# octavian-ganea/equidock_public

Measured on NVIDIA H100. Metric: protein_pairs_per_sec_iegmn_fwd_kabsch, higher is better.
Workload: dtype f32

## Files before the change

### equidock_public_b200/csrc/attn_tc.cu

```cuda
#include "tc_common.cuh"

namespace eqd {

#ifdef ATTN_PROF
__device__ long long g_attn_prof[16];
#define PROF_MARK(k) do { if (tid == 0 && blockIdx.x == 0) { const long long t_ = clock64(); prof_acc[k] += t_ - prof_t; prof_t = t_; } } while (0)
#else
#define PROF_MARK(k) do { } while (0)
#endif

#define AT_THREADS 256
#define AT_KEYS 64
#define AT_CHUNK_BYTES 8192
#define AT_A_SPLIT 16384
#define AT_LD 68

struct AtGroupSmem {
  unsigned char k[2][3][AT_CHUNK_BYTES];
  unsigned char v[2][3][AT_CHUNK_BYTES];
  float red[EQD_TM * 2];
  float x5c[2][AT_KEYS * 16];
  float red5[EQD_TM * 2 * 5];
};
struct AtSmem {
  unsigned char qa[3 * AT_A_SPLIT];
  unsigned char pa[3 * AT_A_SPLIT];
  AtGroupSmem grp;
  unsigned long long k_bar[2], v_bar[2];
};

__global__ void __launch_bounds__(AT_THREADS, 1)
attention0_tc_kernel(eqd_graph g, const float* __restrict__ proj, int pw, const unsigned char* __restrict__ kv,
                    long kv_split_stride, const float* __restrict__ x5, float* __restrict__ mu, int ldmu) {
  extern __shared__ __align__(128) unsigned char smem_raw[];
  AtSmem& S = *reinterpret_cast<AtSmem*>(smem_raw);
  const int tid = threadIdx.x, q = tid, half = q >> 7, r = q & 127, wgi = tid >> 7;
  AtGroupSmem& G = S.grp;
  TRACE_START(1);
  if (tid == 0) {
    for (int b = 0; b < 2; ++b) {
      mbar_init(&S.k_bar[b], 1);
      mbar_init(&S.v_bar[b], 1);
    }
    asm volatile("fence.mbarrier_init.release.cluster;" ::: "memory");
  }
  if (q == 0) TRACE_PHASE(1, blockIdx.x, 0, 14);
  __syncthreads();
  if (q == 0) TRACE_PHASE(1, blockIdx.x, 0, 13);
  const unsigned k_saddr = smem_u32(G.k), v_saddr = smem_u32(G.v);
  const unsigned qa_saddr = smem_u32(S.qa), pa_saddr = smem_u32(S.pa);
  float* const dtile = reinterpret_cast<float*>(S.pa);
  unsigned kph[2] = {0, 0}, vph[2] = {0, 0};
  const int B = g.n_pairs;
  const unsigned char* k_g = kv;
  const unsigned char* v_g = kv + 3 * kv_split_stride;

  auto load_chunk = [&](const unsigned char* src, unsigned char (*dst)[AT_CHUNK_BYTES], unsigned long long* bar, int blk0,
                        int x5buf) {
    if (q == 0) {
      const bool with5 = x5buf >= 0;
      mbar_expect_tx(bar, 3 * AT_CHUNK_BYTES + (with5 ? AT_KEYS * 64 : 0));
#pragma unroll
      for (int s = 0; s < 3; ++s) bulk_g2s(dst[s], src + s * kv_split_stride + (long)blk0 * 1024, AT_CHUNK_BYTES, bar);
      if (with5) bulk_g2s(G.x5c[x5buf], x5 + (long)blk0 * 8 * 16, AT_KEYS * 64, bar);
    }
  };
  auto add_s5 = [&](float (&s)[32], const float* xc, const float (&q5)[5]) {
#pragma unroll
    for (int i = 0; i < 32; ++i) {
      const float* row = xc + (half * 32 + i) * 16;
      const float4 k4 = *reinterpret_cast<const float4*>(row);
      const float k8 = row[8];
      s[i] += q5[0] * k4.x + q5[1] * k4.y + q5[2] * k4.z + q5[3] * k4.w + q5[4] * k8;
    }
  };
  auto gemm_s = [&](int kb_, bool hi_only) {
    float d[32];
    wg_gemm6<64>(d, [&](int sp, int kb) { return a_desc_at<EQD_TM>(qa_saddr, AT_A_SPLIT, wgi, sp, kb); },
                 [&](int sp, int kk) { return b_desc_ex(k_saddr + (kb_ * 3 + sp) * AT_CHUNK_BYTES + kk * 256, 128, 1024); },
                 4, false, hi_only);
    wg_store_d<64>(dtile + wgi * 64 * AT_LD, AT_LD, d, tid & 127);
  };
  auto gemm_pv = [&](int vb_) {
    float d[32];
    wg_gemm6<64, 1>(d, [&](int sp, int kb) { return a_desc_at<EQD_TM>(pa_saddr, AT_A_SPLIT, wgi, sp, kb); },
                    [&](int sp, int kk) { return b_desc_ex(v_saddr + (vb_ * 3 + sp) * AT_CHUNK_BYTES + kk * 2048, 1024, 128); },
                    4, false);
    __syncthreads();
    wg_store_d<64>(dtile + wgi * 64 * AT_LD, AT_LD, d, tid & 127);
  };

#ifdef ATTN_PROF
  __shared__ long long prof_acc[16];
  long long prof_t = clock64();
  if (tid == 0)
    for (int k = 0; k < 16; ++k) prof_acc[k] = 0;
#endif
  for (int tile = blockIdx.x; tile < g.n_node_tiles; tile += gridDim.x) {
    PROF_MARK(15);
    if (q == 0) TRACE_PHASE(1, blockIdx.x, tile, 1);
    const int seg = g.node_tiles[2 * tile], node0 = g.node_tiles[2 * tile + 1];
    const int nvalid = min(EQD_TM, g.seg_ptr[seg + 1] - node0);
    const int pseg = seg < B ? seg + B : seg - B;
    const int j0 = g.seg_ptr[pseg], j1 = g.seg_ptr[pseg + 1];
    const int blk_lo = j0 >> 3, blk_hi = (j1 + 7) >> 3;
    const int nchunks = (blk_hi - blk_lo + 7) >> 3;
    const int node = node0 + r;
    const bool valid = r < nvalid;
    PROF_MARK(0);
    if (nchunks > 0) load_chunk(k_g, G.k[0], &S.k_bar[0], blk_lo, 0);
    float q5[5] = {0.f, 0.f, 0.f, 0.f, 0.f};
    if (valid) {
#pragma unroll
      for (int e = 0; e < 5; ++e) q5[e] = x5[(long)node * 16 + 10 + e];
    }
    {
      float v[32];
      const float4* sp = reinterpret_cast<const float4*>(proj + (long)node * pw + 128 + half * 32);
#pragma unroll
      for (int c4 = 0; c4 < 8; ++c4) {
        float4 t = valid ? sp[c4] : make_float4(0.f, 0.f, 0.f, 0.f);
        v[c4 * 4] = t.x; v[c4 * 4 + 1] = t.y; v[c4 * 4 + 2] = t.z; v[c4 * 4 + 3] = t.w;
      }
      store_half_split3<EQD_TM>(S.qa, AT_A_SPLIT, r, half * 32, v);
    }
    tc_fence_before();
    __syncthreads();
    PROF_MARK(1);
    float mx = -INFINITY;
    for (int c = 0; c < nchunks; ++c) {
      const int kb_ = c & 1;
      if (q == 0) TRACE_PHASE(1, blockIdx.x, tile, (c << 4) | 2);
      mbar_wait(&S.k_bar[kb_], kph[kb_]);
      kph[kb_] ^= 1;
      PROF_MARK(2);
      if (c + 1 < nchunks) load_chunk(k_g, G.k[kb_ ^ 1], &S.k_bar[kb_ ^ 1], blk_lo + 8 * (c + 1), kb_ ^ 1);
      else load_chunk(k_g, G.k[kb_ ^ 1], &S.k_bar[kb_ ^ 1], blk_lo, kb_ ^ 1);
      if (q == 0) TRACE_PHASE(1, blockIdx.x, tile, (c << 4) | 3);
      gemm_s(kb_, true);
      __syncthreads();
      PROF_MARK(3);
      float s[32];
      tile_ld32f(dtile, AT_LD, r, half * 32, s);
      add_s5(s, G.x5c[kb_], q5);
      const int key0 = (blk_lo + 8 * c) * 8 + half * 32;
#pragma unroll
      for (int i = 0; i < 32; ++i) {
        int kn = key0 + i;
        mx = fmaxf(mx, (kn >= j0 && kn < j1) ? s[i] : -INFINITY);
      }
      __syncthreads();
      PROF_MARK(4);
    }
    G.red[r * 2 + half] = mx;
    __syncthreads();
    mx = fmaxf(G.red[r * 2], G.red[r * 2 + 1]);
    float l = 0.f;
    float o_acc[32];
#pragma unroll
    for (int i = 0; i < 32; ++i) o_acc[i] = 0.f;
    if (nchunks > 0) load_chunk(v_g, G.v[0], &S.v_bar[0], blk_lo, -1);
    float o5[5] = {0.f, 0.f, 0.f, 0.f, 0.f};
    for (int c = 0; c < nchunks; ++c) {
      const int kb_ = (nchunks + c) & 1, vb_ = c & 1;
      if (q == 0) TRACE_PHASE(1, blockIdx.x, tile, (c << 4) | 4);
      mbar_wait(&S.k_bar[kb_], kph[kb_]);
      kph[kb_] ^= 1;
      PROF_MARK(5);
      if (c + 1 < nchunks) {
        load_chunk(k_g, G.k[kb_ ^ 1], &S.k_bar[kb_ ^ 1], blk_lo + 8 * (c + 1), kb_ ^ 1);
        load_chunk(v_g, G.v[vb_ ^ 1], &S.v_bar[vb_ ^ 1], blk_lo + 8 * (c + 1), -1);
      }
      if (q == 0) TRACE_PHASE(1, blockIdx.x, tile, (c << 4) | 5);
      gemm_s(kb_, false);
      __syncthreads();
      PROF_MARK(6);
      float s[32];
      tile_ld32f(dtile, AT_LD, r, half * 32, s);
      add_s5(s, G.x5c[kb_], q5);
      const int key0 = (blk_lo + 8 * c) * 8 + half * 32;
      float l4[4] = {0.f, 0.f, 0.f, 0.f};
#pragma unroll
      for (int i = 0; i < 32; ++i) {
        int kn = key0 + i;
        float pj = (kn >= j0 && kn < j1) ? expf(s[i] - mx) : 0.f;
        s[i] = pj;
        l4[i & 3] += pj;
        {
          const float* row = G.x5c[kb_] + (half * 32 + i) * 16;
          const float4 v4 = *reinterpret_cast<const float4*>(row + 4);
          o5[0] = fmaf(pj, v4.x, o5[0]);
          o5[1] = fmaf(pj, v4.y, o5[1]);
          o5[2] = fmaf(pj, v4.z, o5[2]);
          o5[3] = fmaf(pj, v4.w, o5[3]);
          o5[4] = fmaf(pj, row[9], o5[4]);
        }
      }
      l += (l4[0] + l4[1]) + (l4[2] + l4[3]);
      PROF_MARK(7);
      __syncthreads();
      PROF_MARK(8);
      store_half_split3<EQD_TM>(S.pa, AT_A_SPLIT, r, half * 32, s);
      tc_fence_before();
      __syncthreads();
      PROF_MARK(9);
      if (q == 0) TRACE_PHASE(1, blockIdx.x, tile, (c << 4) | 6);
      mbar_wait(&S.v_bar[vb_], vph[vb_]);
      vph[vb_] ^= 1;
      gemm_pv(vb_);
      __syncthreads();
      if (q == 0) TRACE_PHASE(1, blockIdx.x, tile, (c << 4) | 7);
      PROF_MARK(10);
      {
        float oc[32];
        tile_ld32f(dtile, AT_LD, r, half * 32, oc);
#pragma unroll
        for (int i = 0; i < 32; ++i) o_acc[i] += oc[i];
      }
      __syncthreads();
      PROF_MARK(11);
    }
    G.red[r * 2 + half] = l;
    {
#pragma unroll
      for (int e = 0; e < 5; ++e) G.red5[(r * 2 + half) * 5 + e] = o5[e];
    }
    __syncthreads();
    l = G.red[r * 2] + G.red[r * 2 + 1];
    {
      const float inv = l > 0.f ? 1.f / l : 0.f;
      if (valid && half == 0) {
        float e8[8];
#pragma unroll
        for (int e = 0; e < 5; ++e) e8[e] = (G.red5[r * 10 + e] + G.red5[r * 10 + 5 + e]) * inv;
        e8[5] = e8[6] = e8[7] = 0.f;
        float4* de = reinterpret_cast<float4*>(mu + (long)node * ldmu + 64);
        de[0] = make_float4(e8[0], e8[1], e8[2], e8[3]);
        de[1] = make_float4(e8[4], e8[5], e8[6], e8[7]);
      }
      if (valid) {
        float4* dst = reinterpret_cast<float4*>(mu + (long)node * ldmu + half * 32);
#pragma unroll
        for (int c4 = 0; c4 < 8; ++c4)
          dst[c4] = make_float4(o_acc[c4 * 4] * inv, o_acc[c4 * 4 + 1] * inv, o_acc[c4 * 4 + 2] * inv, o_acc[c4 * 4 + 3] * inv);
      }
    }
    __syncthreads();
    PROF_MARK(12);
  }
#ifdef ATTN_PROF
  if (tid == 0 && blockIdx.x == 0)
    for (int k = 0; k < 16; ++k) g_attn_prof[k] = prof_acc[k];
#endif
  if (q == 0) TRACE_PHASE(1, blockIdx.x, 0xffff, 15);
  TRACE_END(1);
}

#define AT_CHAINS 2

struct __align__(128) AtChainSmem {
  unsigned char k[2][3][AT_CHUNK_BYTES];
  unsigned char v[2][3][AT_CHUNK_BYTES];
  float qs[64 * 64];
  unsigned long long k_bar[2], v_bar[2];
};

struct AtTile {
  int node0, nvalid;
  int j0, j1;
  int blk_lo, nchunks;
};

__global__ void __launch_bounds__(AT_CHAINS * 128, 1)
attention64_tc_kernel(eqd_graph g, const float* __restrict__ proj, const unsigned char* __restrict__ kv,
                      long kv_split_stride, float* __restrict__ mu) {
  extern __shared__ __align__(128) unsigned char smem_raw[];
  AtChainSmem& W = reinterpret_cast<AtChainSmem*>(smem_raw)[threadIdx.x >> 7];
  const int tid = threadIdx.x, wgi = tid >> 7, t = tid & 127, lane = t & 31;
  const int bar = 1 + wgi;
  TRACE_START(1);
  if (t == 0) {
    for (int b = 0; b < 2; ++b) {
      mbar_init(&W.k_bar[b], 1);
      mbar_init(&W.v_bar[b], 1);
    }
    asm volatile("fence.mbarrier_init.release.cluster;" ::: "memory");
  }
  wg_barrier(bar);
  const unsigned k_saddr = smem_u32(W.k), v_saddr = smem_u32(W.v);
  const int B = g.n_pairs, nht = 2 * g.n_node_tiles, hstride = gridDim.x * AT_CHAINS;
  const unsigned char* k_g = kv;
  const unsigned char* v_g = kv + 3 * kv_split_stride;

  const int chain = blockIdx.x * AT_CHAINS + wgi;
  auto find_tile = [&](int k, AtTile& m) {
    for (; chain + k * hstride < nht; ++k) {
      const int ht = (chain + k * hstride) ^ (k & 1);
      const int seg = __ldg(g.node_tiles + 2 * (ht >> 1));
      m.node0 = __ldg(g.node_tiles + 2 * (ht >> 1) + 1) + 64 * (ht & 1);
      m.nvalid = min(64, __ldg(g.seg_ptr + seg + 1) - m.node0);
      if (m.nvalid <= 0) continue;
      const int pseg = seg < B ? seg + B : seg - B;
      m.j0 = __ldg(g.seg_ptr + pseg);
      m.j1 = __ldg(g.seg_ptr + pseg + 1);
      m.blk_lo = m.j0 >> 3;
      m.nchunks = (((m.j1 + 7) >> 3) - m.blk_lo + 7) >> 3;
      return k;
    }
    return -1;
  };
  unsigned kfill = 0, kcons = 0, vfill = 0, vcons = 0;
  auto fill = [&](unsigned char (*dst)[3][AT_CHUNK_BYTES], unsigned long long* bars, unsigned& n, const unsigned char* src,
                  int blk0) {
    if (t == 0) {
      unsigned long long* b = &bars[n & 1];
      mbar_expect_tx(b, 3 * AT_CHUNK_BYTES);
#pragma unroll
      for (int s = 0; s < 3; ++s) bulk_g2s(dst[n & 1][s], src + s * kv_split_stride + (long)blk0 * 1024, AT_CHUNK_BYTES, b);
    }
    ++n;
  };
  auto consume = [&](unsigned long long* bars, unsigned& n) {
    mbar_wait(&bars[n & 1], (n >> 1) & 1);
    return (int)((n++) & 1);
  };
  auto stage_q = [&](const AtTile& m) { stage_rows64(W.qs, proj, 320, 128, m.node0, m.nvalid, t); };

  const int fr0 = (t >> 5) * 16 + (lane >> 2), fc = 2 * (lane & 3);
  AtTile cur, nxt;
  int kt = find_tile(0, cur);
  bool k_ahead = false, v_ahead = false;
  if (kt >= 0) stage_q(cur);
  while (kt >= 0) {
    if (t == 0) TRACE_PHASE(1, chain, kt, 1);
    int ktn = -1;
    bool looked = false;
    auto look_ahead = [&]() {
      if (looked) return;
      looked = true;
      ktn = find_tile(kt + 1, nxt);
      if (ktn >= 0) stage_q(nxt);
    };
    if (cur.nchunks > 0 && !k_ahead) fill(W.k, W.k_bar, kfill, k_g, cur.blk_lo);
    cp_async_wait<0>();
    wg_barrier(bar);
    unsigned qf[3][4][4];
    staged_rows_to_a_split3(W.qs, t, qf);
    wg_barrier(bar);
    auto k_desc = [&](int kb_) {
      return [&, kb_](int sp, int kk) { return b_desc_ex(k_saddr + (kb_ * 3 + sp) * AT_CHUNK_BYTES + kk * 256, 128, 1024); };
    };
    float mx[2] = {-INFINITY, -INFINITY};
    for (int c = 0; c < cur.nchunks; ++c) {
      const int kb_ = consume(W.k_bar, kcons);
      fill(W.k, W.k_bar, kfill, k_g, cur.blk_lo + (c + 1 < cur.nchunks ? 8 * (c + 1) : 0));
      float s[32];
      wg_gemm6_rs_issue<64, 4, 0, true>(s, qf, k_desc(kb_), false);
      look_ahead();
      wg_mma_wait(s);
      const int key0 = (cur.blk_lo + 8 * c) * 8 + fc;
#pragma unroll
      for (int j = 0; j < 8; ++j)
#pragma unroll
        for (int e = 0; e < 2; ++e) {
          const int kn = key0 + 8 * j + e;
          const bool ok = kn >= cur.j0 && kn < cur.j1;
#pragma unroll
          for (int h = 0; h < 2; ++h) mx[h] = fmaxf(mx[h], ok ? s[4 * j + 2 * h + e] : -INFINITY);
        }
      wg_barrier(bar);
    }
    look_ahead();
#pragma unroll
    for (int h = 0; h < 2; ++h) {
      mx[h] = fmaxf(mx[h], __shfl_xor_sync(0xffffffffu, mx[h], 1));
      mx[h] = fmaxf(mx[h], __shfl_xor_sync(0xffffffffu, mx[h], 2));
    }
    float lh[2][2] = {{0.f, 0.f}, {0.f, 0.f}};
    float o_acc[32];
#pragma unroll
    for (int i = 0; i < 32; ++i) o_acc[i] = 0.f;
    if (cur.nchunks > 0 && !v_ahead) fill(W.v, W.v_bar, vfill, v_g, cur.blk_lo);
    for (int c = 0; c < cur.nchunks; ++c) {
      const int kb_ = consume(W.k_bar, kcons);
      const bool last = c + 1 == cur.nchunks;
      if (!last) {
        fill(W.k, W.k_bar, kfill, k_g, cur.blk_lo + 8 * (c + 1));
        fill(W.v, W.v_bar, vfill, v_g, cur.blk_lo + 8 * (c + 1));
      } else if (ktn >= 0 && nxt.nchunks > 0) {
        fill(W.k, W.k_bar, kfill, k_g, nxt.blk_lo);
        fill(W.v, W.v_bar, vfill, v_g, nxt.blk_lo);
      }
      float s[32];
      wg_gemm6_rs_issue<64, 4>(s, qf, k_desc(kb_), false);
      wg_mma_wait(s);
      const int key0 = (cur.blk_lo + 8 * c) * 8 + fc;
#pragma unroll
      for (int j = 0; j < 8; ++j)
#pragma unroll
        for (int e = 0; e < 2; ++e) {
          const int kn = key0 + 8 * j + e;
          const bool ok = kn >= cur.j0 && kn < cur.j1;
#pragma unroll
          for (int h = 0; h < 2; ++h) {
            float& x = s[4 * j + 2 * h + e];
            x = ok ? expf(x - mx[h]) : 0.f;
          }
        }
      {
        float ps[32];
#pragma unroll
        for (int i = 0; i < 32; ++i) ps[i] = __shfl_xor_sync(0xffffffffu, s[i], 2);
#pragma unroll
        for (int h = 0; h < 2; ++h)
#pragma unroll
          for (int ch = 0; ch < 2; ++ch) {
            float s0 = 0.f, s1 = 0.f;
#pragma unroll
            for (int c4 = 0; c4 < 8; ++c4) {
              s0 = __fadd_rn(s0, chain_val(s, ps, h, ch, c4, 0));
              s1 = __fadd_rn(s1, chain_val(s, ps, h, ch, c4, 1));
            }
            const float sp = __fadd_rn(s0, s1);
            lh[h][ch] = __fadd_rn(lh[h][ch], __fadd_rn(sp, __shfl_xor_sync(0xffffffffu, sp, 1)));
          }
      }
      unsigned pf[3][4][4];
      acc_to_a_split3<4>(s, pf);
      const int vb_ = consume(W.v_bar, vcons);
      float o[32];
      wg_gemm6_rs_issue<64, 4, 1>(o, pf, [&](int sp, int kk) {
        return b_desc_ex(v_saddr + (vb_ * 3 + sp) * AT_CHUNK_BYTES + kk * 2048, 1024, 128); }, false);
      wg_mma_wait(o);
#pragma unroll
      for (int i = 0; i < 32; ++i) o_acc[i] = __fadd_rn(o_acc[i], o[i]);
      wg_barrier(bar);
    }
    k_ahead = v_ahead = ktn >= 0 && nxt.nchunks > 0 && cur.nchunks > 0;
#pragma unroll
    for (int h = 0; h < 2; ++h) {
      const float l = __fadd_rn(lh[h][0], lh[h][1]);
      const float inv = l > 0.f ? 1.f / l : 0.f;
      const int row = fr0 + 8 * h;
      if (row < cur.nvalid) {
        float* dst = mu + (long)(cur.node0 + row) * EQD_HID + fc;
#pragma unroll
        for (int j = 0; j < 8; ++j)
          *reinterpret_cast<float2*>(dst + 8 * j) = make_float2(o_acc[4 * j + 2 * h] * inv, o_acc[4 * j + 2 * h + 1] * inv);
      }
    }
    kt = ktn;
    cur = nxt;
  }
  cp_async_wait<0>();
  TRACE_END(1);
}

}

EQD_TRACE_SETTER(eqd_trace_set_attn)

#ifdef ATTN_PROF
extern "C" int eqd_attn_prof_read(long long* out16) {
  return (int)cudaMemcpyFromSymbol(out16, eqd::g_attn_prof, sizeof(long long) * 16);
}
#endif

extern "C" int eqd_attention_tc(const eqd_graph* g, const float* proj, const void* kv, float* mu, void* stream) {
  if (!g || !proj || !kv || !mu) return EQD_ERR_BAD_ARG;
  if (reinterpret_cast<uintptr_t>(kv) & 15) return EQD_ERR_BAD_ARG;
  if (g->n_node_tiles <= 0) return EQD_OK;
  const size_t smem = AT_CHAINS * sizeof(eqd::AtChainSmem);
  EQD_SET_SMEM(eqd::attention64_tc_kernel, smem);
  const int nht = 2 * g->n_node_tiles;
  int grid = (nht + AT_CHAINS - 1) / AT_CHAINS;
  if (grid > EQD_SMS) grid = EQD_SMS;
  const long split_stride = (long)((g->n_nodes + 7) / 8 + 8) * 1024;
  eqd::attention64_tc_kernel<<<grid, AT_CHAINS * 128, smem, (cudaStream_t)stream>>>(
      *g, proj, reinterpret_cast<const unsigned char*>(kv), split_stride, mu);
  EQD_CUDA_LAUNCH_CHECK();
  return EQD_OK;
}

extern "C" int eqd_attention_tc0(const eqd_graph* g, const float* proj, const void* kv, const float* x5, float* mu,
                                 void* stream) {
  if (!g || !proj || !kv || !x5 || !mu) return EQD_ERR_BAD_ARG;
  if ((reinterpret_cast<uintptr_t>(kv) | reinterpret_cast<uintptr_t>(x5)) & 15) return EQD_ERR_BAD_ARG;
  if (g->n_node_tiles <= 0) return EQD_OK;
  const size_t smem = sizeof(eqd::AtSmem) + 128;
  EQD_SET_SMEM(eqd::attention0_tc_kernel, smem);
  const int grid = g->n_node_tiles < EQD_SMS ? g->n_node_tiles : EQD_SMS;
  const long split_stride = (long)((g->n_nodes + 7) / 8 + 8) * 1024;
  eqd::attention0_tc_kernel<<<grid, AT_THREADS, smem, (cudaStream_t)stream>>>(
      *g, proj, 128 + 3 * 72, reinterpret_cast<const unsigned char*>(kv), split_stride, x5, mu, EQD_H0_PAD);
  EQD_CUDA_LAUNCH_CHECK();
  return EQD_OK;
}
```

### equidock_public_b200/csrc/tc_common.cuh

```cuda
#pragma once
#include "common.cuh"

namespace eqd {

__device__ __forceinline__ unsigned smem_u32(const void* p) { return (unsigned)__cvta_generic_to_shared(p); }

__device__ __forceinline__ void mbar_init(unsigned long long* bar, int count) {
  asm volatile("mbarrier.init.shared::cta.b64 [%0], %1;" ::"r"(smem_u32(bar)), "r"(count));
}
__device__ __forceinline__ void mbar_wait(unsigned long long* bar, unsigned parity) {
  unsigned addr = smem_u32(bar);
  unsigned done = 0;
  while (!done) {
    asm volatile(
        "{\n\t.reg .pred p;\n\t"
        "mbarrier.try_wait.parity.shared::cta.b64 p, [%1], %2;\n\t"
        "selp.u32 %0, 1, 0, p;\n\t}"
        : "=r"(done) : "r"(addr), "r"(parity) : "memory");
  }
}
__device__ __forceinline__ void mbar_expect_tx(unsigned long long* bar, unsigned bytes) {
  asm volatile("mbarrier.arrive.expect_tx.shared::cta.b64 _, [%0], %1;" ::"r"(smem_u32(bar)), "r"(bytes) : "memory");
}
__device__ __forceinline__ void bulk_g2s(void* dst, const void* src, unsigned bytes, unsigned long long* bar) {
  asm volatile("cp.async.bulk.shared::cluster.global.mbarrier::complete_tx::bytes [%0], [%1], %2, [%3];" ::"r"(smem_u32(dst)),
               "l"(src), "r"(bytes), "r"(smem_u32(bar)) : "memory");
}
__device__ __forceinline__ void cp_async8(void* dst, const void* src) {
  asm volatile("cp.async.ca.shared.global [%0], [%1], 8;" ::"r"(smem_u32(dst)), "l"(src));
}
__device__ __forceinline__ void cp_async4(void* dst, const void* src) {
  asm volatile("cp.async.ca.shared.global [%0], [%1], 4;" ::"r"(smem_u32(dst)), "l"(src));
}
__device__ __forceinline__ void tc_fence_before() { asm volatile("fence.proxy.async.shared::cta;" ::: "memory"); }

__device__ __forceinline__ unsigned long long b_desc_ex(unsigned saddr, unsigned lbo, unsigned sbo) {
  return (unsigned long long)((saddr >> 4) & 0x3FFF) | ((unsigned long long)((lbo >> 4) & 0x3FFF) << 16) |
         ((unsigned long long)((sbo >> 4) & 0x3FFF) << 32);
}

template <int N, int TB>
struct Wgmma;
template <int TB>
struct Wgmma<16, TB> {
  static __device__ __forceinline__ void mma(float (&d)[8], unsigned long long a, unsigned long long b, int scale_d) {
    asm volatile(
        "{\n\t.reg .pred p;\n\tsetp.ne.b32 p, %10, 0;\n\t"
        "wgmma.mma_async.sync.aligned.m64n16k16.f32.bf16.bf16 {%0, %1, %2, %3, %4, %5, %6, %7}, %8, %9, p, 1, 1, 0, %11;\n\t}"
        : "+f"(d[0]), "+f"(d[1]), "+f"(d[2]), "+f"(d[3]), "+f"(d[4]), "+f"(d[5]), "+f"(d[6]), "+f"(d[7])
        : "l"(a), "l"(b), "r"(scale_d), "n"(TB));
  }
};
template <int TB>
struct Wgmma<64, TB> {
  static __device__ __forceinline__ void mma(float (&d)[32], unsigned long long a, unsigned long long b, int scale_d) {
    asm volatile(
        "{\n\t.reg .pred p;\n\tsetp.ne.b32 p, %34, 0;\n\t"
        "wgmma.mma_async.sync.aligned.m64n64k16.f32.bf16.bf16 {%0, %1, %2, %3, %4, %5, %6, %7, %8, %9, %10, %11, %12, %13, %14, %15, %16, %17, %18, %19, %20, %21, %22, %23, %24, %25, %26, %27, %28, %29, %30, %31}, %32, %33, p, 1, 1, 0, %35;\n\t}"
        : "+f"(d[0]), "+f"(d[1]), "+f"(d[2]), "+f"(d[3]), "+f"(d[4]), "+f"(d[5]), "+f"(d[6]), "+f"(d[7]), "+f"(d[8]), "+f"(d[9]), "+f"(d[10]), "+f"(d[11]), "+f"(d[12]), "+f"(d[13]), "+f"(d[14]), "+f"(d[15]), "+f"(d[16]), "+f"(d[17]), "+f"(d[18]), "+f"(d[19]), "+f"(d[20]), "+f"(d[21]), "+f"(d[22]), "+f"(d[23]), "+f"(d[24]), "+f"(d[25]), "+f"(d[26]), "+f"(d[27]), "+f"(d[28]), "+f"(d[29]), "+f"(d[30]), "+f"(d[31])
        : "l"(a), "l"(b), "r"(scale_d), "n"(TB));
  }
};
template <int TB>
struct Wgmma<80, TB> {
  static __device__ __forceinline__ void mma(float (&d)[40], unsigned long long a, unsigned long long b, int scale_d) {
    asm volatile(
        "{\n\t.reg .pred p;\n\tsetp.ne.b32 p, %42, 0;\n\t"
        "wgmma.mma_async.sync.aligned.m64n80k16.f32.bf16.bf16 {%0, %1, %2, %3, %4, %5, %6, %7, %8, %9, %10, %11, %12, %13, %14, %15, %16, %17, %18, %19, %20, %21, %22, %23, %24, %25, %26, %27, %28, %29, %30, %31, %32, %33, %34, %35, %36, %37, %38, %39}, %40, %41, p, 1, 1, 0, %43;\n\t}"
        : "+f"(d[0]), "+f"(d[1]), "+f"(d[2]), "+f"(d[3]), "+f"(d[4]), "+f"(d[5]), "+f"(d[6]), "+f"(d[7]), "+f"(d[8]), "+f"(d[9]), "+f"(d[10]), "+f"(d[11]), "+f"(d[12]), "+f"(d[13]), "+f"(d[14]), "+f"(d[15]), "+f"(d[16]), "+f"(d[17]), "+f"(d[18]), "+f"(d[19]), "+f"(d[20]), "+f"(d[21]), "+f"(d[22]), "+f"(d[23]), "+f"(d[24]), "+f"(d[25]), "+f"(d[26]), "+f"(d[27]), "+f"(d[28]), "+f"(d[29]), "+f"(d[30]), "+f"(d[31]), "+f"(d[32]), "+f"(d[33]), "+f"(d[34]), "+f"(d[35]), "+f"(d[36]), "+f"(d[37]), "+f"(d[38]), "+f"(d[39])
        : "l"(a), "l"(b), "r"(scale_d), "n"(TB));
  }
};

template <int N, int TB>
struct WgmmaRS;
template <int TB>
struct WgmmaRS<64, TB> {
  static __device__ __forceinline__ void mma(float (&d)[32], const unsigned (&a)[4], unsigned long long b, int scale_d) {
    asm volatile(
        "{\n\t.reg .pred p;\n\tsetp.ne.b32 p, %37, 0;\n\t"
        "wgmma.mma_async.sync.aligned.m64n64k16.f32.bf16.bf16 {%0, %1, %2, %3, %4, %5, %6, %7, %8, %9, %10, %11, %12, %13, %14, %15, %16, %17, %18, %19, %20, %21, %22, %23, %24, %25, %26, %27, %28, %29, %30, %31}, {%32, %33, %34, %35}, %36, p, 1, 1, %38;\n\t}"
        : "+f"(d[0]), "+f"(d[1]), "+f"(d[2]), "+f"(d[3]), "+f"(d[4]), "+f"(d[5]), "+f"(d[6]), "+f"(d[7]), "+f"(d[8]), "+f"(d[9]), "+f"(d[10]), "+f"(d[11]), "+f"(d[12]), "+f"(d[13]), "+f"(d[14]), "+f"(d[15]), "+f"(d[16]), "+f"(d[17]), "+f"(d[18]), "+f"(d[19]), "+f"(d[20]), "+f"(d[21]), "+f"(d[22]), "+f"(d[23]), "+f"(d[24]), "+f"(d[25]), "+f"(d[26]), "+f"(d[27]), "+f"(d[28]), "+f"(d[29]), "+f"(d[30]), "+f"(d[31])
        : "r"(a[0]), "r"(a[1]), "r"(a[2]), "r"(a[3]), "l"(b), "r"(scale_d), "n"(TB));
  }
};

template <int N, int TB = 0, class AD, class BD>
__device__ __forceinline__ void wg_gemm6_issue(float (&d)[N / 2], AD a_desc, BD b_desc, int kblocks, bool accumulate,
                                               bool hi_only = false) {
  const int pa[6] = {2, 0, 1, 1, 0, 0}, pb[6] = {0, 2, 1, 0, 1, 0};
  asm volatile("wgmma.fence.sync.aligned;" ::: "memory");
  int scale_d = accumulate ? 1 : 0;
#pragma unroll
  for (int pr = hi_only ? 5 : 0; pr < 6; ++pr)
    for (int kb = 0; kb < kblocks; ++kb) {
      Wgmma<N, TB>::mma(d, a_desc(pa[pr], kb), b_desc(pb[pr], kb), scale_d);
      scale_d = 1;
    }
  asm volatile("wgmma.commit_group.sync.aligned;" ::: "memory");
}
template <int PENDING = 0, int M>
__device__ __forceinline__ void wg_mma_wait(float (&d)[M]) {
  asm volatile("wgmma.wait_group.sync.aligned %0;" ::"n"(PENDING) : "memory");
#pragma unroll
  for (int i = 0; i < M; ++i) asm volatile("" : "+f"(d[i])::"memory");
}
template <int N, int TB = 0, class AD, class BD>
__device__ __forceinline__ void wg_gemm6(float (&d)[N / 2], AD a_desc, BD b_desc, int kblocks, bool accumulate,
                                         bool hi_only = false) {
  wg_gemm6_issue<N, TB>(d, a_desc, b_desc, kblocks, accumulate, hi_only);
  asm volatile("wgmma.wait_group.sync.aligned 0;" ::: "memory");
}
template <int N, int KB, int TB = 0, bool HI_ONLY = false, class BD>
__device__ __forceinline__ void wg_gemm6_rs_issue(float (&d)[N / 2], const unsigned (&a)[3][KB][4], BD b_desc, bool accumulate) {
  constexpr int pa[6] = {2, 0, 1, 1, 0, 0}, pb[6] = {0, 2, 1, 0, 1, 0};
  asm volatile("wgmma.fence.sync.aligned;" ::: "memory");
  int scale_d = accumulate ? 1 : 0;
#pragma unroll
  for (int pr = HI_ONLY ? 5 : 0; pr < 6; ++pr)
#pragma unroll
    for (int kb = 0; kb < KB; ++kb) {
      WgmmaRS<N, TB>::mma(d, a[pa[pr]][kb], b_desc(pb[pr], kb), scale_d);
      scale_d = 1;
    }
  asm volatile("wgmma.commit_group.sync.aligned;" ::: "memory");
}

template <int R>
__device__ __forceinline__ unsigned long long a_desc_at(unsigned a_saddr, unsigned split_bytes, int wgi, int s, int kb) {
  return b_desc_ex(a_saddr + s * split_bytes + kb * (32 * R) + wgi * 1024, 16 * R, 128);
}
template <int R>
__device__ __forceinline__ void a_store8(unsigned char* a, unsigned split_bytes, int row, int c, const unsigned* p0,
                                         const unsigned* p1, const unsigned* p2) {
  unsigned char* base = a + (c >> 4) * (32 * R) + ((c >> 3) & 1) * (16 * R) + (row >> 3) * 128 + (row & 7) * 16;
  *reinterpret_cast<uint4*>(base) = make_uint4(p0[0], p0[1], p0[2], p0[3]);
  *reinterpret_cast<uint4*>(base + split_bytes) = make_uint4(p1[0], p1[1], p1[2], p1[3]);
  *reinterpret_cast<uint4*>(base + 2 * split_bytes) = make_uint4(p2[0], p2[1], p2[2], p2[3]);
}

template <int N>
__device__ __forceinline__ void wg_store_d(float* tile, int ld, const float (&d)[N / 2], int t) {
  const int row = (t >> 5) * 16 + ((t & 31) >> 2), col = 2 * (t & 3);
#pragma unroll
  for (int j = 0; j < N / 8; ++j) {
    *reinterpret_cast<float2*>(tile + row * ld + 8 * j + col) = make_float2(d[4 * j], d[4 * j + 1]);
    *reinterpret_cast<float2*>(tile + (row + 8) * ld + 8 * j + col) = make_float2(d[4 * j + 2], d[4 * j + 3]);
  }
}

__device__ __forceinline__ unsigned cvt_bf16x2(float hi, float lo) {
  unsigned d;
  asm("cvt.rn.bf16x2.f32 %0, %1, %2;" : "=r"(d) : "f"(hi), "f"(lo));
  return d;
}
__device__ __forceinline__ void split3_pair(float v0, float v1, unsigned& p0, unsigned& p1, unsigned& p2) {
  p0 = cvt_bf16x2(v1, v0);
  const float r0 = v0 - __uint_as_float(p0 << 16), r1 = v1 - __uint_as_float(p0 & 0xFFFF0000u);
  p1 = cvt_bf16x2(r1, r0);
  p2 = cvt_bf16x2(r1 - __uint_as_float(p1 & 0xFFFF0000u), r0 - __uint_as_float(p1 << 16));
}
template <int R>
__device__ __forceinline__ void store_half_split3(unsigned char* a, unsigned split_bytes, int row, int c0, const float (&v)[32]) {
  unsigned p0[16], p1[16], p2[16];
#pragma unroll
  for (int c = 0; c < 16; ++c) split3_pair(v[2 * c], v[2 * c + 1], p0[c], p1[c], p2[c]);
#pragma unroll
  for (int j = 0; j < 4; ++j) a_store8<R>(a, split_bytes, row, c0 + 8 * j, p0 + 4 * j, p1 + 4 * j, p2 + 4 * j);
}
template <int R>
__device__ __forceinline__ void store_extra8_split3(unsigned char* a, unsigned split_bytes, int row, int c0, const float (&t)[8]) {
  unsigned p0[8], p1[8], p2[8];
#pragma unroll
  for (int c = 0; c < 4; ++c) split3_pair(t[2 * c], t[2 * c + 1], p0[c], p1[c], p2[c]);
#pragma unroll
  for (int c = 4; c < 8; ++c) p0[c] = p1[c] = p2[c] = 0u;
  a_store8<R>(a, split_bytes, row, c0, p0, p1, p2);
  a_store8<R>(a, split_bytes, row, c0 + 8, p0 + 4, p1 + 4, p2 + 4);
}
template <int KB>
__device__ __forceinline__ void acc_to_a_split3(const float (&v)[8 * KB], unsigned (&a)[3][KB][4]) {
#pragma unroll
  for (int kb = 0; kb < KB; ++kb)
#pragma unroll
    for (int i = 0; i < 4; ++i) split3_pair(v[8 * kb + 2 * i], v[8 * kb + 2 * i + 1], a[0][kb][i], a[1][kb][i], a[2][kb][i]);
}
__device__ __forceinline__ int stage_swz(int row) { return (row & 3) << 1; }
__device__ __forceinline__ void stage_rows64(float* rows, const float* src, int ld, int col0, long row0, int nvalid, int t) {
#pragma unroll
  for (int i = 0; i < 8; ++i) {
    const int idx = i * 128 + t, row = idx >> 4, k4 = idx & 15;
    const bool ok = row < nvalid;
    cp_async16(rows + row * 64 + ((k4 ^ stage_swz(row)) << 2), src + (row0 + (ok ? row : 0)) * ld + col0 + 4 * k4, ok);
  }
  cp_async_commit();
}
__device__ __forceinline__ void staged_rows_to_a_split3(const float* rows, int t, unsigned (&a)[3][4][4]) {
  const int g = (t >> 5) * 16 + ((t & 31) >> 2), c = t & 3;
#pragma unroll
  for (int kb = 0; kb < 4; ++kb)
#pragma unroll
    for (int i = 0; i < 4; ++i) {
      const int row = g + 8 * (i & 1), k4 = 4 * kb + 2 * (i >> 1) + (c >> 1);
      const float2 v = *reinterpret_cast<const float2*>(rows + row * 64 + ((k4 ^ stage_swz(row)) << 2) + 2 * (c & 1));
      split3_pair(v.x, v.y, a[0][kb][i], a[1][kb][i], a[2][kb][i]);
    }
}
__device__ __forceinline__ void staged_rows_to_frag(const float* rows, int t, float (&v)[32]) {
  const int g = (t >> 5) * 16 + ((t & 31) >> 2), c = t & 3;
#pragma unroll
  for (int kb = 0; kb < 4; ++kb)
#pragma unroll
    for (int i = 0; i < 4; ++i) {
      const int row = g + 8 * (i & 1), k4 = 4 * kb + 2 * (i >> 1) + (c >> 1);
      const float2 x = *reinterpret_cast<const float2*>(rows + row * 64 + ((k4 ^ stage_swz(row)) << 2) + 2 * (c & 1));
      v[8 * kb + 2 * i] = x.x;
      v[8 * kb + 2 * i + 1] = x.y;
    }
}
__device__ __forceinline__ float chain_val(const float (&v)[32], const float (&pv)[32], int h, int ch, int c4, int e) {
  const int i = 4 * (4 * ch + (c4 >> 1)) + 2 * h + e;
  const bool own = ((c4 & 1) == 0) == ((threadIdx.x & 2) == 0);
  return own ? v[i] : pv[i];
}
__device__ __forceinline__ void wg_barrier(int id) { asm volatile("bar.sync %0, 128;" ::"r"(id) : "memory"); }
__device__ __forceinline__ bool wg_barrier_and(int id, bool pred) {
  unsigned all;
  asm volatile(
      "{\n\t.reg .pred p, q;\n\tsetp.ne.u32 p, %1, 0;\n\t"
      "bar.red.and.pred q, %2, 128, p;\n\tselp.u32 %0, 1, 0, q;\n\t}"
      : "=r"(all) : "r"((unsigned)pred), "r"(id) : "memory");
  return all != 0;
}
__device__ __forceinline__ void tile_ld32f(const float* tile, int ld, int row, int c0, float (&v)[32]) {
  const float4* s = reinterpret_cast<const float4*>(tile + row * ld + c0);
#pragma unroll
  for (int c4 = 0; c4 < 8; ++c4) {
    float4 t = s[c4];
    v[c4 * 4] = t.x; v[c4 * 4 + 1] = t.y; v[c4 * 4 + 2] = t.z; v[c4 * 4 + 3] = t.w;
  }
}

}
```

Measured before the change: 34820.

## Trim last key chunk loads and wgmma widths to valid 16-key steps

Computes how many 16-key steps of the final chunk per segment are actually valid and uses that to shrink the TMA bulk copies and select narrower wgmma N shapes (16/32/48) for the score and PV GEMMs via a runtime switch. The first max-pass also loads only the hi split of K when only the hi-only product is needed. This aims to cut wasted memory traffic and tensor-core work on partially filled tail chunks, at the cost of more code paths and a runtime dispatch per chunk.

```diff
diff --git a/equidock_public_b200/csrc/attn_tc.cu b/equidock_public_b200/csrc/attn_tc.cu
--- a/equidock_public_b200/csrc/attn_tc.cu
+++ b/equidock_public_b200/csrc/attn_tc.cu
@@ -14,6 +14,10 @@
 #define AT_CHUNK_BYTES 8192
 #define AT_A_SPLIT 16384
 #define AT_LD 68
+
+__device__ __forceinline__ int at_last_steps(int blk_lo, int nchunks, int j1) {
+  return (j1 - (blk_lo + 8 * (nchunks - 1)) * 8 + 15) >> 4;
+}
 
 struct AtGroupSmem {
   unsigned char k[2][3][AT_CHUNK_BYTES];
@@ -56,13 +60,12 @@
   const unsigned char* v_g = kv + 3 * kv_split_stride;
 
   auto load_chunk = [&](const unsigned char* src, unsigned char (*dst)[AT_CHUNK_BYTES], unsigned long long* bar, int blk0,
-                        int x5buf) {
+                        int x5buf, int nsplit, int steps) {
     if (q == 0) {
       const bool with5 = x5buf >= 0;
-      mbar_expect_tx(bar, 3 * AT_CHUNK_BYTES + (with5 ? AT_KEYS * 64 : 0));
-#pragma unroll
-      for (int s = 0; s < 3; ++s) bulk_g2s(dst[s], src + s * kv_split_stride + (long)blk0 * 1024, AT_CHUNK_BYTES, bar);
-      if (with5) bulk_g2s(G.x5c[x5buf], x5 + (long)blk0 * 8 * 16, AT_KEYS * 64, bar);
+      mbar_expect_tx(bar, (nsplit * 2048 + (with5 ? 16 * 64 : 0)) * steps);
+      for (int s = 0; s < nsplit; ++s) bulk_g2s(dst[s], src + s * kv_split_stride + (long)blk0 * 1024, steps * 2048, bar);
+      if (with5) bulk_g2s(G.x5c[x5buf], x5 + (long)blk0 * 8 * 16, steps * 16 * 64, bar);
     }
   };
   auto add_s5 = [&](float (&s)[32], const float* xc, const float (&q5)[5]) {
@@ -74,18 +77,23 @@
       s[i] += q5[0] * k4.x + q5[1] * k4.y + q5[2] * k4.z + q5[3] * k4.w + q5[4] * k8;
     }
   };
-  auto gemm_s = [&](int kb_, bool hi_only) {
+  auto gemm_s = [&](int kb_, bool hi_only, int steps) {
+    with_steps(steps, [&](auto ns) {
+      constexpr int n = 16 * decltype(ns)::value;
+      float d[n / 2];
+      wg_gemm6<n>(d, [&](int sp, int kb) { return a_desc_at<EQD_TM>(qa_saddr, AT_A_SPLIT, wgi, sp, kb); },
+                  [&](int sp, int kk) { return b_desc_ex(k_saddr + (kb_ * 3 + sp) * AT_CHUNK_BYTES + kk * 256, 128, 1024); },
+                  4, false, hi_only);
+      wg_store_d<n>(dtile + wgi * 64 * AT_LD, AT_LD, d, tid & 127);
+    });
+  };
+  auto gemm_pv = [&](int vb_, int steps) {
     float d[32];
-    wg_gemm6<64>(d, [&](int sp, int kb) { return a_desc_at<EQD_TM>(qa_saddr, AT_A_SPLIT, wgi, sp, kb); },
-                 [&](int sp, int kk) { return b_desc_ex(k_saddr + (kb_ * 3 + sp) * AT_CHUNK_BYTES + kk * 256, 128, 1024); },
-                 4, false, hi_only);
-    wg_store_d<64>(dtile + wgi * 64 * AT_LD, AT_LD, d, tid & 127);
-  };
-  auto gemm_pv = [&](int vb_) {
-    float d[32];
-    wg_gemm6<64, 1>(d, [&](int sp, int kb) { return a_desc_at<EQD_TM>(pa_saddr, AT_A_SPLIT, wgi, sp, kb); },
-                    [&](int sp, int kk) { return b_desc_ex(v_saddr + (vb_ * 3 + sp) * AT_CHUNK_BYTES + kk * 2048, 1024, 128); },
-                    4, false);
+    with_steps(steps, [&](auto ns) {
+      wg_gemm6<64, 1>(d, [&](int sp, int kb) { return a_desc_at<EQD_TM>(pa_saddr, AT_A_SPLIT, wgi, sp, kb); },
+                      [&](int sp, int kk) { return b_desc_ex(v_saddr + (vb_ * 3 + sp) * AT_CHUNK_BYTES + kk * 2048, 1024, 128); },
+                      decltype(ns)::value, false);
+    });
     __syncthreads();
     wg_store_d<64>(dtile + wgi * 64 * AT_LD, AT_LD, d, tid & 127);
   };
@@ -105,10 +113,12 @@
     const int j0 = g.seg_ptr[pseg], j1 = g.seg_ptr[pseg + 1];
     const int blk_lo = j0 >> 3, blk_hi = (j1 + 7) >> 3;
     const int nchunks = (blk_hi - blk_lo + 7) >> 3;
+    const int last_steps = at_last_steps(blk_lo, nchunks, j1);
+    auto steps = [&](int c) { return c + 1 < nchunks ? 4 : last_steps; };
     const int node = node0 + r;
     const bool valid = r < nvalid;
     PROF_MARK(0);
-    if (nchunks > 0) load_chunk(k_g, G.k[0], &S.k_bar[0], blk_lo, 0);
+    if (nchunks > 0) load_chunk(k_g, G.k[0], &S.k_bar[0], blk_lo, 0, 1, 4);
     float q5[5] = {0.f, 0.f, 0.f, 0.f, 0.f};
     if (valid) {
 #pragma unroll
@@ -134,10 +144,10 @@
       mbar_wait(&S.k_bar[kb_], kph[kb_]);
       kph[kb_] ^= 1;
       PROF_MARK(2);
-      if (c + 1 < nchunks) load_chunk(k_g, G.k[kb_ ^ 1], &S.k_bar[kb_ ^ 1], blk_lo + 8 * (c + 1), kb_ ^ 1);
-      else load_chunk(k_g, G.k[kb_ ^ 1], &S.k_bar[kb_ ^ 1], blk_lo, kb_ ^ 1);
+      if (c + 1 < nchunks) load_chunk(k_g, G.k[kb_ ^ 1], &S.k_bar[kb_ ^ 1], blk_lo + 8 * (c + 1), kb_ ^ 1, 1, 4);
+      else load_chunk(k_g, G.k[kb_ ^ 1], &S.k_bar[kb_ ^ 1], blk_lo, kb_ ^ 1, 3, steps(0));
       if (q == 0) TRACE_PHASE(1, blockIdx.x, tile, (c << 4) | 3);
-      gemm_s(kb_, true);
+      gemm_s(kb_, true, 4);
       __syncthreads();
       PROF_MARK(3);
       float s[32];
@@ -159,20 +169,21 @@
     float o_acc[32];
 #pragma unroll
     for (int i = 0; i < 32; ++i) o_acc[i] = 0.f;
-    if (nchunks > 0) load_chunk(v_g, G.v[0], &S.v_bar[0], blk_lo, -1);
+    if (nchunks > 0) load_chunk(v_g, G.v[0], &S.v_bar[0], blk_lo, -1, 3, steps(0));
     float o5[5] = {0.f, 0.f, 0.f, 0.f, 0.f};
     for (int c = 0; c < nchunks; ++c) {
       const int kb_ = (nchunks + c) & 1, vb_ = c & 1;
+      const int ns = steps(c);
       if (q == 0) TRACE_PHASE(1, blockIdx.x, tile, (c << 4) | 4);
       mbar_wait(&S.k_bar[kb_], kph[kb_]);
       kph[kb_] ^= 1;
       PROF_MARK(5);
       if (c + 1 < nchunks) {
-        load_chunk(k_g, G.k[kb_ ^ 1], &S.k_bar[kb_ ^ 1], blk_lo + 8 * (c + 1), kb_ ^ 1);
-        load_chunk(v_g, G.v[vb_ ^ 1], &S.v_bar[vb_ ^ 1], blk_lo + 8 * (c + 1), -1);
+        load_chunk(k_g, G.k[kb_ ^ 1], &S.k_bar[kb_ ^ 1], blk_lo + 8 * (c + 1), kb_ ^ 1, 3, steps(c + 1));
+        load_chunk(v_g, G.v[vb_ ^ 1], &S.v_bar[vb_ ^ 1], blk_lo + 8 * (c + 1), -1, 3, steps(c + 1));
       }
       if (q == 0) TRACE_PHASE(1, blockIdx.x, tile, (c << 4) | 5);
-      gemm_s(kb_, false);
+      gemm_s(kb_, false, ns);
       __syncthreads();
       PROF_MARK(6);
       float s[32];
@@ -186,7 +197,7 @@
         float pj = (kn >= j0 && kn < j1) ? expf(s[i] - mx) : 0.f;
         s[i] = pj;
         l4[i & 3] += pj;
-        {
+        if (half * 32 + i < 16 * ns) {
           const float* row = G.x5c[kb_] + (half * 32 + i) * 16;
           const float4 v4 = *reinterpret_cast<const float4*>(row + 4);
           o5[0] = fmaf(pj, v4.x, o5[0]);
@@ -207,7 +218,7 @@
       if (q == 0) TRACE_PHASE(1, blockIdx.x, tile, (c << 4) | 6);
       mbar_wait(&S.v_bar[vb_], vph[vb_]);
       vph[vb_] ^= 1;
-      gemm_pv(vb_);
+      gemm_pv(vb_, ns);
       __syncthreads();
       if (q == 0) TRACE_PHASE(1, blockIdx.x, tile, (c << 4) | 7);
       PROF_MARK(10);
@@ -269,6 +280,8 @@
   int node0, nvalid;
   int j0, j1;
   int blk_lo, nchunks;
+  int last_steps;
+  __device__ int steps(int c) const { return c + 1 < nchunks ? 4 : last_steps; }
 };
 
 __global__ void __launch_bounds__(AT_CHAINS * 128, 1)
@@ -305,18 +318,19 @@
       m.j1 = __ldg(g.seg_ptr + pseg + 1);
       m.blk_lo = m.j0 >> 3;
       m.nchunks = (((m.j1 + 7) >> 3) - m.blk_lo + 7) >> 3;
+      m.last_steps = at_last_steps(m.blk_lo, m.nchunks, m.j1);
       return k;
     }
     return -1;
   };
   unsigned kfill = 0, kcons = 0, vfill = 0, vcons = 0;
   auto fill = [&](unsigned char (*dst)[3][AT_CHUNK_BYTES], unsigned long long* bars, unsigned& n, const unsigned char* src,
-                  int blk0) {
+                  int blk0, int nsplit, int steps) {
     if (t == 0) {
       unsigned long long* b = &bars[n & 1];
-      mbar_expect_tx(b, 3 * AT_CHUNK_BYTES);
-#pragma unroll
-      for (int s = 0; s < 3; ++s) bulk_g2s(dst[n & 1][s], src + s * kv_split_stride + (long)blk0 * 1024, AT_CHUNK_BYTES, b);
+      mbar_expect_tx(b, nsplit * steps * 2048);
+      for (int s = 0; s < nsplit; ++s)
+        bulk_g2s(dst[n & 1][s], src + s * kv_split_stride + (long)blk0 * 1024, steps * 2048, b);
     }
     ++n;
   };
@@ -341,7 +355,7 @@
       ktn = find_tile(kt + 1, nxt);
       if (ktn >= 0) stage_q(nxt);
     };
-    if (cur.nchunks > 0 && !k_ahead) fill(W.k, W.k_bar, kfill, k_g, cur.blk_lo);
+    if (cur.nchunks > 0 && !k_ahead) fill(W.k, W.k_bar, kfill, k_g, cur.blk_lo, 1, 4);
     cp_async_wait<0>();
     wg_barrier(bar);
     unsigned qf[3][4][4];
@@ -353,7 +367,8 @@
     float mx[2] = {-INFINITY, -INFINITY};
     for (int c = 0; c < cur.nchunks; ++c) {
       const int kb_ = consume(W.k_bar, kcons);
-      fill(W.k, W.k_bar, kfill, k_g, cur.blk_lo + (c + 1 < cur.nchunks ? 8 * (c + 1) : 0));
+      if (c + 1 < cur.nchunks) fill(W.k, W.k_bar, kfill, k_g, cur.blk_lo + 8 * (c + 1), 1, 4);
+      else fill(W.k, W.k_bar, kfill, k_g, cur.blk_lo, 3, cur.steps(0));
       float s[32];
       wg_gemm6_rs_issue<64, 4, 0, true>(s, qf, k_desc(kb_), false);
       look_ahead();
@@ -380,20 +395,26 @@
     float o_acc[32];
 #pragma unroll
     for (int i = 0; i < 32; ++i) o_acc[i] = 0.f;
-    if (cur.nchunks > 0 && !v_ahead) fill(W.v, W.v_bar, vfill, v_g, cur.blk_lo);
+    if (cur.nchunks > 0 && !v_ahead) fill(W.v, W.v_bar, vfill, v_g, cur.blk_lo, 3, cur.steps(0));
     for (int c = 0; c < cur.nchunks; ++c) {
       const int kb_ = consume(W.k_bar, kcons);
       const bool last = c + 1 == cur.nchunks;
+      const int ns = cur.steps(c);
       if (!last) {
-        fill(W.k, W.k_bar, kfill, k_g, cur.blk_lo + 8 * (c + 1));
-        fill(W.v, W.v_bar, vfill, v_g, cur.blk_lo + 8 * (c + 1));
+        fill(W.k, W.k_bar, kfill, k_g, cur.blk_lo + 8 * (c + 1), 3, cur.steps(c + 1));
+        fill(W.v, W.v_bar, vfill, v_g, cur.blk_lo + 8 * (c + 1), 3, cur.steps(c + 1));
       } else if (ktn >= 0 && nxt.nchunks > 0) {
-        fill(W.k, W.k_bar, kfill, k_g, nxt.blk_lo);
-        fill(W.v, W.v_bar, vfill, v_g, nxt.blk_lo);
+        fill(W.k, W.k_bar, kfill, k_g, nxt.blk_lo, 1, 4);
+        fill(W.v, W.v_bar, vfill, v_g, nxt.blk_lo, 3, nxt.steps(0));
       }
       float s[32];
-      wg_gemm6_rs_issue<64, 4>(s, qf, k_desc(kb_), false);
-      wg_mma_wait(s);
+#pragma unroll
+      for (int i = 0; i < 32; ++i) s[i] = 0.f;
+      with_steps(ns, [&](auto n_) {
+        constexpr int n = decltype(n_)::value;
+        wg_gemm6_rs_issue<16 * n, 4>(frag_head<8 * n>(s), qf, k_desc(kb_), false);
+        wg_mma_wait(frag_head<8 * n>(s));
+      });
       const int key0 = (cur.blk_lo + 8 * c) * 8 + fc;
 #pragma unroll
       for (int j = 0; j < 8; ++j)
@@ -429,9 +450,11 @@
       acc_to_a_split3<4>(s, pf);
       const int vb_ = consume(W.v_bar, vcons);
       float o[32];
-      wg_gemm6_rs_issue<64, 4, 1>(o, pf, [&](int sp, int kk) {
-        return b_desc_ex(v_saddr + (vb_ * 3 + sp) * AT_CHUNK_BYTES + kk * 2048, 1024, 128); }, false);
-      wg_mma_wait(o);
+      with_steps(ns, [&](auto n_) {
+        wg_gemm6_rs_issue<64, decltype(n_)::value, 1>(o, pf, [&](int sp, int kk) {
+          return b_desc_ex(v_saddr + (vb_ * 3 + sp) * AT_CHUNK_BYTES + kk * 2048, 1024, 128); }, false);
+        wg_mma_wait(o);
+      });
 #pragma unroll
       for (int i = 0; i < 32; ++i) o_acc[i] = __fadd_rn(o_acc[i], o[i]);
       wg_barrier(bar);
diff --git a/equidock_public_b200/csrc/tc_common.cuh b/equidock_public_b200/csrc/tc_common.cuh
--- a/equidock_public_b200/csrc/tc_common.cuh
+++ b/equidock_public_b200/csrc/tc_common.cuh
@@ -52,6 +52,26 @@
   }
 };
 template <int TB>
+struct Wgmma<32, TB> {
+  static __device__ __forceinline__ void mma(float (&d)[16], unsigned long long a, unsigned long long b, int scale_d) {
+    asm volatile(
+        "{\n\t.reg .pred p;\n\tsetp.ne.b32 p, %18, 0;\n\t"
+        "wgmma.mma_async.sync.aligned.m64n32k16.f32.bf16.bf16 {%0, %1, %2, %3, %4, %5, %6, %7, %8, %9, %10, %11, %12, %13, %14, %15}, %16, %17, p, 1, 1, 0, %19;\n\t}"
+        : "+f"(d[0]), "+f"(d[1]), "+f"(d[2]), "+f"(d[3]), "+f"(d[4]), "+f"(d[5]), "+f"(d[6]), "+f"(d[7]), "+f"(d[8]), "+f"(d[9]), "+f"(d[10]), "+f"(d[11]), "+f"(d[12]), "+f"(d[13]), "+f"(d[14]), "+f"(d[15])
+        : "l"(a), "l"(b), "r"(scale_d), "n"(TB));
+  }
+};
+template <int TB>
+struct Wgmma<48, TB> {
+  static __device__ __forceinline__ void mma(float (&d)[24], unsigned long long a, unsigned long long b, int scale_d) {
+    asm volatile(
+        "{\n\t.reg .pred p;\n\tsetp.ne.b32 p, %26, 0;\n\t"
+        "wgmma.mma_async.sync.aligned.m64n48k16.f32.bf16.bf16 {%0, %1, %2, %3, %4, %5, %6, %7, %8, %9, %10, %11, %12, %13, %14, %15, %16, %17, %18, %19, %20, %21, %22, %23}, %24, %25, p, 1, 1, 0, %27;\n\t}"
+        : "+f"(d[0]), "+f"(d[1]), "+f"(d[2]), "+f"(d[3]), "+f"(d[4]), "+f"(d[5]), "+f"(d[6]), "+f"(d[7]), "+f"(d[8]), "+f"(d[9]), "+f"(d[10]), "+f"(d[11]), "+f"(d[12]), "+f"(d[13]), "+f"(d[14]), "+f"(d[15]), "+f"(d[16]), "+f"(d[17]), "+f"(d[18]), "+f"(d[19]), "+f"(d[20]), "+f"(d[21]), "+f"(d[22]), "+f"(d[23])
+        : "l"(a), "l"(b), "r"(scale_d), "n"(TB));
+  }
+};
+template <int TB>
 struct Wgmma<64, TB> {
   static __device__ __forceinline__ void mma(float (&d)[32], unsigned long long a, unsigned long long b, int scale_d) {
     asm volatile(
@@ -74,6 +94,36 @@
 
 template <int N, int TB>
 struct WgmmaRS;
+template <int TB>
+struct WgmmaRS<16, TB> {
+  static __device__ __forceinline__ void mma(float (&d)[8], const unsigned (&a)[4], unsigned long long b, int scale_d) {
+    asm volatile(
+        "{\n\t.reg .pred p;\n\tsetp.ne.b32 p, %13, 0;\n\t"
+        "wgmma.mma_async.sync.aligned.m64n16k16.f32.bf16.bf16 {%0, %1, %2, %3, %4, %5, %6, %7}, {%8, %9, %10, %11}, %12, p, 1, 1, %14;\n\t}"
+        : "+f"(d[0]), "+f"(d[1]), "+f"(d[2]), "+f"(d[3]), "+f"(d[4]), "+f"(d[5]), "+f"(d[6]), "+f"(d[7])
+        : "r"(a[0]), "r"(a[1]), "r"(a[2]), "r"(a[3]), "l"(b), "r"(scale_d), "n"(TB));
+  }
+};
+template <int TB>
+struct WgmmaRS<32, TB> {
+  static __device__ __forceinline__ void mma(float (&d)[16], const unsigned (&a)[4], unsigned long long b, int scale_d) {
+    asm volatile(
+        "{\n\t.reg .pred p;\n\tsetp.ne.b32 p, %21, 0;\n\t"
+        "wgmma.mma_async.sync.aligned.m64n32k16.f32.bf16.bf16 {%0, %1, %2, %3, %4, %5, %6, %7, %8, %9, %10, %11, %12, %13, %14, %15}, {%16, %17, %18, %19}, %20, p, 1, 1, %22;\n\t}"
+        : "+f"(d[0]), "+f"(d[1]), "+f"(d[2]), "+f"(d[3]), "+f"(d[4]), "+f"(d[5]), "+f"(d[6]), "+f"(d[7]), "+f"(d[8]), "+f"(d[9]), "+f"(d[10]), "+f"(d[11]), "+f"(d[12]), "+f"(d[13]), "+f"(d[14]), "+f"(d[15])
+        : "r"(a[0]), "r"(a[1]), "r"(a[2]), "r"(a[3]), "l"(b), "r"(scale_d), "n"(TB));
+  }
+};
+template <int TB>
+struct WgmmaRS<48, TB> {
+  static __device__ __forceinline__ void mma(float (&d)[24], const unsigned (&a)[4], unsigned long long b, int scale_d) {
+    asm volatile(
+        "{\n\t.reg .pred p;\n\tsetp.ne.b32 p, %29, 0;\n\t"
+        "wgmma.mma_async.sync.aligned.m64n48k16.f32.bf16.bf16 {%0, %1, %2, %3, %4, %5, %6, %7, %8, %9, %10, %11, %12, %13, %14, %15, %16, %17, %18, %19, %20, %21, %22, %23}, {%24, %25, %26, %27}, %28, p, 1, 1, %30;\n\t}"
+        : "+f"(d[0]), "+f"(d[1]), "+f"(d[2]), "+f"(d[3]), "+f"(d[4]), "+f"(d[5]), "+f"(d[6]), "+f"(d[7]), "+f"(d[8]), "+f"(d[9]), "+f"(d[10]), "+f"(d[11]), "+f"(d[12]), "+f"(d[13]), "+f"(d[14]), "+f"(d[15]), "+f"(d[16]), "+f"(d[17]), "+f"(d[18]), "+f"(d[19]), "+f"(d[20]), "+f"(d[21]), "+f"(d[22]), "+f"(d[23])
+        : "r"(a[0]), "r"(a[1]), "r"(a[2]), "r"(a[3]), "l"(b), "r"(scale_d), "n"(TB));
+  }
+};
 template <int TB>
 struct WgmmaRS<64, TB> {
   static __device__ __forceinline__ void mma(float (&d)[32], const unsigned (&a)[4], unsigned long long b, int scale_d) {
@@ -111,8 +161,10 @@
   wg_gemm6_issue<N, TB>(d, a_desc, b_desc, kblocks, accumulate, hi_only);
   asm volatile("wgmma.wait_group.sync.aligned 0;" ::: "memory");
 }
-template <int N, int KB, int TB = 0, bool HI_ONLY = false, class BD>
-__device__ __forceinline__ void wg_gemm6_rs_issue(float (&d)[N / 2], const unsigned (&a)[3][KB][4], BD b_desc, bool accumulate) {
+template <int N, int KB_ = 0, int TB = 0, bool HI_ONLY = false, class BD, int KBA>
+__device__ __forceinline__ void wg_gemm6_rs_issue(float (&d)[N / 2], const unsigned (&a)[3][KBA][4], BD b_desc, bool accumulate) {
+  constexpr int KB = KB_ > 0 ? KB_ : KBA;
+  static_assert(KB <= KBA, "more k-blocks than A fragments");
   constexpr int pa[6] = {2, 0, 1, 1, 0, 0}, pb[6] = {0, 2, 1, 0, 1, 0};
   asm volatile("wgmma.fence.sync.aligned;" ::: "memory");
   int scale_d = accumulate ? 1 : 0;
@@ -124,6 +176,27 @@
       scale_d = 1;
     }
   asm volatile("wgmma.commit_group.sync.aligned;" ::: "memory");
+}
+
+template <int M>
+using FragRegs = float[M];
+template <int M, int L>
+__device__ __forceinline__ FragRegs<M>& frag_head(float (&v)[L]) {
+  static_assert(M <= L, "head longer than the fragment");
+  return *reinterpret_cast<FragRegs<M>*>(&v[0]);
+}
+template <int V>
+struct IntConst {
+  static constexpr int value = V;
+};
+template <class F>
+__device__ __forceinline__ void with_steps(int steps, F&& f) {
+  switch (steps) {
+    case 1: f(IntConst<1>{}); break;
+    case 2: f(IntConst<2>{}); break;
+    case 3: f(IntConst<3>{}); break;
+    default: f(IntConst<4>{}); break;
+  }
 }
 
 template <int R>
```

Result: faster. 35690, median of 6 (+2.5%).
